# wsntxxn/TextToAudioGrounding

Hardware: AMD Instinct MI355X
Metric: clips/sec (10 s@32 kHz, 1-phrase) fwd+bwd (higher is better)
Workload: dtype f32

## Files before the change

### texttoaudiogrounding_amd/csrc/conv_wino.hip

```cpp
#include "conv_wino.h"

int tag_launch_gemm_batched(const float* A, int lda, long sA, const float* B, int ldb, long sB, float* C, int ldc, long sC, int M,
                            int N, int K, int batch, hipStream_t st, int transA);

namespace {

__device__ __forceinline__ f32x4 wino_prologue(f32x4 v, int mode, f32x4 s, f32x4 t) {
    if (mode == 1) {
        v.x = fmaxf(fmaf(v.x, s.x, t.x), 0.0f); v.y = fmaxf(fmaf(v.y, s.y, t.y), 0.0f);
        v.z = fmaxf(fmaf(v.z, s.z, t.z), 0.0f); v.w = fmaxf(fmaf(v.w, s.w, t.w), 0.0f);
    } else if (mode == 2) {
        v.x = fmaf(v.x > 0 ? v.x : 0.1f * v.x, s.x, t.x); v.y = fmaf(v.y > 0 ? v.y : 0.1f * v.y, s.y, t.y);
        v.z = fmaf(v.z > 0 ? v.z : 0.1f * v.z, s.z, t.z); v.w = fmaf(v.w > 0 ? v.w : 0.1f * v.w, s.w, t.w);
    } else if (mode == 3) {
        v.x = fmaf(v.x, s.x, t.x); v.y = fmaf(v.y, s.y, t.y); v.z = fmaf(v.z, s.z, t.z); v.w = fmaf(v.w, s.w, t.w);
    }
    return v;
}

__global__ __launch_bounds__(256) void wino_pack_kernel(const float* __restrict__ w, float* __restrict__ Uf,
                                                        float* __restrict__ Ud, int Cin, int Cout, int tiled_f, int tiled_d) {
    const long n = (long)Cin * Cout;
    for (long e = (long)blockIdx.x * 256 + threadIdx.x; e < n; e += (long)gridDim.x * 256) {
        const int co = (int)(e / Cin), ci = (int)(e % Cin);
// ... 318 lines not shown
        float q[3][4];
#pragma unroll
        for (int s = 0; s < 4; ++s) {
            const float hs = 0.5f * (u[1][s] + u[2][s]), hd = 0.5f * (u[1][s] - u[2][s]);
            q[0][s] = u[0][s] + hs;
            q[1][s] = hd;
            q[2][s] = hs + u[3][s];
        }
        float* o = dw + e * 9;
#pragma unroll
        for (int a = 0; a < 3; ++a) {
            const float hs = 0.5f * (q[a][1] + q[a][2]), hd = 0.5f * (q[a][1] - q[a][2]);
            o[3 * a + 0] = q[a][0] + hs;
            o[3 * a + 1] = hd;
            o[3 * a + 2] = hs + q[a][3];
        }
    }
}

struct WinoWgGeom { int th, tw; long T, Tpad; int S, kc; };
inline WinoWgGeom wino_wg_geom(int B, int H, int W, int Cin, int Cout) {
    WinoWgGeom g;
    g.th = (H + 1) / 2; g.tw = (W + 1) / 2;
    g.T = (long)B * g.th * g.tw;
    const long tiles = (long)((Cin + 127) / 128) * ((Cout + 127) / 128) * 16;
    long S = (1024 + tiles - 1) / tiles;
    if (S > g.T / 512) S = g.T / 512;
    if (S < 1) S = 1;
    long kc = (g.T + S - 1) / S;
    kc = (kc + 15) / 16 * 16;
    g.S = (int)((g.T + kc - 1) / kc);
    g.kc = (int)kc;
    g.Tpad = (long)g.S * kc;
    return g;
}

struct WinoGeom { int th, tw; long T; int G, P; };
inline WinoGeom wino_geom(int B, int H, int W, int Cout) {
    WinoGeom g;
    g.th = (H + 1) / 2; g.tw = (W + 1) / 2;
    g.T = (long)B * g.th * g.tw;
    g.G = 256 / (Cout / 4);
    const long per_wg = (long)g.G * WINO_ITERS;
    g.P = (int)((g.T + per_wg - 1) / per_wg) * g.G;
    return g;
}
inline bool wino_channels_ok(int C) { return C >= 32 && C <= 1024 && C % 4 == 0 && 256 % (C / 4) == 0; }

int wino_run(const float* x, const float* U, int pro, const float* s, const float* t, float* y, float* stats, const WinoEpi* epi,
             int B, int H, int W, int Cin, int Cout, float* ws, hipStream_t st, float* v_keep = nullptr) {
    if (wino_fused_ok(Cin, Cout)) {
        if (v_keep) {
            const WinoGeom gk = wino_geom(B, H, W, Cout);
            const int gk_in = (int)((gk.T * (Cin / 4) + 255) / 256);
            switch (pro) {
                case 0: hipLaunchKernelGGL(wino_input_kernel<0>, dim3(gk_in), dim3(256), 0, st, x, s, t, v_keep, B, H, W, Cin, gk.th, gk.tw, gk.T, gk.T); break;
                case 1: hipLaunchKernelGGL(wino_input_kernel<1>, dim3(gk_in), dim3(256), 0, st, x, s, t, v_keep, B, H, W, Cin, gk.th, gk.tw, gk.T, gk.T); break;
                case 2: hipLaunchKernelGGL(wino_input_kernel<2>, dim3(gk_in), dim3(256), 0, st, x, s, t, v_keep, B, H, W, Cin, gk.th, gk.tw, gk.T, gk.T); break;
                default: hipLaunchKernelGGL(wino_input_kernel<3>, dim3(gk_in), dim3(256), 0, st, x, s, t, v_keep, B, H, W, Cin, gk.th, gk.tw, gk.T, gk.T); break;
            }
        }
        return wino_fused_run(x, U, pro, s, t, y, stats, epi, B, H, W, Cin, Cout, st);
    }
    const WinoGeom g = wino_geom(B, H, W, Cout);
    float* V = v_keep ? v_keep : ws;
    float* Mb = v_keep ? ws : ws + (size_t)16 * g.T * Cin;
    const long items = g.T * (Cin / 4);
    const int gin = (int)((items + 255) / 256);
    switch (pro) {
        case 0: hipLaunchKernelGGL(wino_input_kernel<0>, dim3(gin), dim3(256), 0, st, x, s, t, V, B, H, W, Cin, g.th, g.tw, g.T, g.T); break;
        case 1: hipLaunchKernelGGL(wino_input_kernel<1>, dim3(gin), dim3(256), 0, st, x, s, t, V, B, H, W, Cin, g.th, g.tw, g.T, g.T); break;
        case 2: hipLaunchKernelGGL(wino_input_kernel<2>, dim3(gin), dim3(256), 0, st, x, s, t, V, B, H, W, Cin, g.th, g.tw, g.T, g.T); break;
        default: hipLaunchKernelGGL(wino_input_kernel<3>, dim3(gin), dim3(256), 0, st, x, s, t, V, B, H, W, Cin, g.th, g.tw, g.T, g.T); break;
    }
    tag_launch_gemm_batched(V, Cin, g.T * Cin, U, Cout, (long)Cin * Cout, Mb, Cout, g.T * Cout, (int)g.T, Cout, Cin, 16, st, 0);
    const int gout = g.P / g.G;
    const WinoEpi none{nullptr, nullptr, nullptr, nullptr, nullptr, 0, 0.0f, 0.0f, 0, 0, 0.0f, 0ull, 0};
    if (epi && epi->kind == 2)
        hipLaunchKernelGGL(wino_output_kernel<2>, dim3(gout), dim3(256), 0, st, Mb, y, stats, *epi, B, H, W, Cout, g.th, g.tw, g.T, g.P);
    else if (epi && epi->kind == 3)
        hipLaunchKernelGGL(wino_output_kernel<3>, dim3(gout), dim3(256), 0, st, Mb, y, stats, *epi, B, H, W, Cout, g.th, g.tw, g.T, g.P);
    else if (epi)
        hipLaunchKernelGGL(wino_output_kernel<1>, dim3(gout), dim3(256), 0, st, Mb, y, stats, *epi, B, H, W, Cout, g.th, g.tw, g.T, g.P);
    else
        hipLaunchKernelGGL(wino_output_kernel<0>, dim3(gout), dim3(256), 0, st, Mb, y, stats, none, B, H, W, Cout, g.th, g.tw, g.T, g.P);
    return 0;
}

}

extern "C" int tag_conv3x3_wino_ok(int B, int H, int W, int Cin, int Cout) {
    const bool fused = Cin % 64 == 0 && Cout % 64 == 0 && Cin >= 64 && Cout >= 64 && Cin <= 1024 && Cout <= 1024;
    if (!(B > 0 && H > 0 && W > 0 && (fused || (wino_channels_ok(Cin) && wino_channels_ok(Cout) && Cin % 32 == 0)))) return 0;
    const WinoGeom g = wino_geom(B, H, W, Cout);
    return g.T < (1L << 31) / 16 && (long)B * H * W < (1L << 31) && (long)B * H * W * (Cin > Cout ? Cin : Cout) < (1L << 29);
}

extern "C" int tag_pack_conv_weight_wino(const float* w, float* ufwd, float* udgrad, int Cin, int Cout, void* stream) {
    TAG_CHECK_ARG(w && (ufwd || udgrad) && Cin > 0 && Cout > 0);
    const long n = (long)Cin * Cout;
    hipLaunchKernelGGL(wino_pack_kernel, dim3(cdiv(n, 256) > 2048 ? 2048 : cdiv(n, 256)), dim3(256), 0, as_stream(stream), w, ufwd,
                       udgrad, Cin, Cout, wino_fused_ok(Cin, Cout) ? 1 : 0, wino_fused_ok(Cout, Cin) ? 1 : 0);
    TAG_LAUNCH_CHECK();
    return 0;
}

extern "C" size_t tag_conv3x3_wino_ws_bytes(int B, int H, int W, int Cin, int Cout) {
    if (wino_fused_ok(Cin > 0 ? Cin : 32, Cout)) return 64;
    const WinoGeom g = wino_geom(B, H, W, Cout);
    return (size_t)16 * g.T * ((size_t)Cin + Cout) * sizeof(float);
}

extern "C" int tag_conv3x3_wino_stats_rows(int B, int H, int W, int Cout) {
    if (wino_fused_ok(32, Cout)) return wino_fused_rows(B, H, W);
    if (!wino_channels_ok(Cout)) return 0;
    return wino_geom(B, H, W, Cout).P;
}

extern "C" int tag_conv3x3_wino_dgrad_poolsums(const float* dy, const float* u, float* dx, const float* yref, const float* bn_scale,
                                               const float* bn_shift, const float* bn_mean, const float* bn_invstd, float* bnpart,
                                               int B, int H, int W, int Cin, int Cout, int Hf, int Wf, int ph, int pw, int pool,
                                               float drop_p, uint64_t seed, void* ws, void* stream) {
    TAG_CHECK_ARG(dy && u && dx && yref && bn_scale && bn_shift && bn_mean && bn_invstd && bnpart && ws);
    TAG_CHECK_ARG(tag_conv3x3_wino_ok(B, H, W, Cin, Cout) && (long)B * Hf * Wf < (1L << 31));
    TAG_CHECK_ARG(pw == 2 && (ph == 1 || ph == 2) && H == Hf / ph && W == Wf / pw);
    TAG_CHECK_ARG((pool == 0 || pool == 2 || pool == 3) && drop_p >= 0.0f && drop_p < 1.0f);
    const float wavg = pool == 3 ? 0.0f : 1.0f / (float)(ph * pw), wmax = pool == 2 ? 0.0f : 1.0f;
    const WinoEpi epi{yref, bn_scale, bn_shift, bn_mean, bn_invstd, ph, wavg, wmax, Hf, Wf, drop_p, (unsigned long long)seed, 2};
    wino_run(dy, u, 0, nullptr, nullptr, dx, bnpart, &epi, B, H, W, Cin, Cout, static_cast<float*>(ws), as_stream(stream));
    TAG_LAUNCH_CHECK();
    return 0;
}

extern "C" size_t tag_conv3x3_wino_wgrad_ws_bytes(int B, int H, int W, int Cin, int Cout) {
    if (wino_fused_wgrad_ok(Cin, Cout)) return wino_fused_wgrad_ws_floats(B, H, W, Cin, Cout) * sizeof(float);
    const WinoWgGeom g = wino_wg_geom(B, H, W, Cin, Cout);
    return ((size_t)16 * g.Tpad * ((size_t)Cin + Cout) + (size_t)16 * g.S * Cin * Cout) * sizeof(float);
}

extern "C" int tag_conv3x3_wino_wgrad_can_reuse_v(int B, int H, int W, int Cin, int Cout) {
    if (wino_fused_wgrad_ok(Cin, Cout)) return 0;
    const WinoWgGeom g = wino_wg_geom(B, H, W, Cin, Cout);
    return g.Tpad == g.T;
}

extern "C" int tag_conv3x3_wino_wgrad(const float* x, int prologue, const float* in_scale, const float* in_shift, const float* dy,
                                      float* dw, int B, int H, int W, int Cin, int Cout, void* ws, const float* v_saved,
                                      void* stream) {
    TAG_CHECK_ARG((x || v_saved) && dy && dw && ws && tag_conv3x3_wino_ok(B, H, W, Cin, Cout));
    TAG_CHECK_ARG(v_saved == nullptr || tag_conv3x3_wino_wgrad_can_reuse_v(B, H, W, Cin, Cout));
    TAG_CHECK_ARG(prologue >= 0 && prologue <= 3 && (prologue == 0 || (in_scale && in_shift)));
    hipStream_t st = as_stream(stream);
    if (wino_fused_wgrad_ok(Cin, Cout) && x) {
        wino_fused_wgrad_run(x, prologue, in_scale, in_shift, dy, dw, B, H, W, Cin, Cout, static_cast<float*>(ws), st);
        TAG_LAUNCH_CHECK();
        return 0;
    }
    const WinoWgGeom g = wino_wg_geom(B, H, W, Cin, Cout);
    float* D = v_saved ? static_cast<float*>(ws) : static_cast<float*>(ws) + (size_t)16 * g.Tpad * Cin;
    const float* V = v_saved ? v_saved : static_cast<const float*>(ws);
    float* Vw = static_cast<float*>(ws);
    float* Pp = D + (size_t)16 * g.Tpad * Cout;
    const int gin = (int)((g.Tpad * (Cin / 4) + 255) / 256), gdy = (int)((g.Tpad * (Cout / 4) + 255) / 256);
    if (!v_saved) switch (prologue) {
        case 0: hipLaunchKernelGGL(wino_input_kernel<0>, dim3(gin), dim3(256), 0, st, x, in_scale, in_shift, Vw, B, H, W, Cin, g.th, g.tw, g.T, g.Tpad); break;
        case 1: hipLaunchKernelGGL(wino_input_kernel<1>, dim3(gin), dim3(256), 0, st, x, in_scale, in_shift, Vw, B, H, W, Cin, g.th, g.tw, g.T, g.Tpad); break;
        case 2: hipLaunchKernelGGL(wino_input_kernel<2>, dim3(gin), dim3(256), 0, st, x, in_scale, in_shift, Vw, B, H, W, Cin, g.th, g.tw, g.T, g.Tpad); break;
        default: hipLaunchKernelGGL(wino_input_kernel<3>, dim3(gin), dim3(256), 0, st, x, in_scale, in_shift, Vw, B, H, W, Cin, g.th, g.tw, g.T, g.Tpad); break;
    }
    hipLaunchKernelGGL(wino_dy_kernel, dim3(gdy), dim3(256), 0, st, dy, D, B, H, W, Cout, g.th, g.tw, g.T, g.Tpad);
    tag_launch_gemm_batched(D, Cout, (long)g.kc * Cout, V, Cin, (long)g.kc * Cin, Pp, Cin, (long)Cin * Cout, Cout, Cin, g.kc,
                            16 * g.S, st, 1);
    const long n = (long)Cin * Cout;
    hipLaunchKernelGGL(wino_wgrad_finish_kernel, dim3(cdiv(n, 256) > 4096 ? 4096 : cdiv(n, 256)), dim3(256), 0, st, Pp, g.S, Cin, Cout,
                       dw);
    TAG_LAUNCH_CHECK();
    return 0;
}

extern "C" int tag_conv3x3_wino_forward(const float* x, const float* u, int prologue, const float* in_scale,
                                        const float* in_shift, float* y, float* stats, int B, int H, int W, int Cin, int Cout,
                                        void* ws, float* v_keep, void* stream) {
    TAG_CHECK_ARG(x && u && y && ws && tag_conv3x3_wino_ok(B, H, W, Cin, Cout));
    TAG_CHECK_ARG(prologue >= 0 && prologue <= 3 && (prologue == 0 || (in_scale && in_shift)));
    wino_run(x, u, prologue, in_scale, in_shift, y, stats, nullptr, B, H, W, Cin, Cout, static_cast<float*>(ws), as_stream(stream),
             v_keep);
    TAG_LAUNCH_CHECK();
    return 0;
}

extern "C" int tag_conv3x3_wino_forward_bnrelu_pool_eval(const float* x, const float* u, int prologue, const float* in_scale,
                                                         const float* in_shift, float* out, const float* bn_scale,
                                                         const float* bn_shift, int B, int H, int W, int Cin, int Cout, int ph, int pw,
                                                         int pool, void* ws, void* stream) {
    TAG_CHECK_ARG(x && u && out && bn_scale && bn_shift && ws && tag_conv3x3_wino_ok(B, H, W, Cin, Cout));
    TAG_CHECK_ARG(prologue >= 0 && prologue <= 3 && (prologue == 0 || (in_scale && in_shift)));
    TAG_CHECK_ARG(pw == 2 && (ph == 1 || ph == 2) && H / ph > 0 && W >= 2 && (pool == 0 || pool == 2 || pool == 3));
    const float wavg = pool == 3 ? 0.0f : 1.0f / (float)(ph * pw), wmax = pool == 2 ? 0.0f : 1.0f;
    const WinoEpi epi{nullptr, bn_scale, bn_shift, nullptr, nullptr, ph, wavg, wmax, 0, 0, 0.0f, 0ull, 3};
    wino_run(x, u, prologue, in_scale, in_shift, out, nullptr, &epi, B, H, W, Cin, Cout, static_cast<float*>(ws), as_stream(stream));
    TAG_LAUNCH_CHECK();
    return 0;
}

extern "C" int tag_conv3x3_wino_dgrad_bnsums(const float* dy, const float* u, float* da, const float* yref, const float* bn_scale,
                                             const float* bn_shift, const float* bn_mean, const float* bn_invstd, float* bnpart,
                                             int B, int H, int W, int Cin, int Cout, void* ws, void* stream) {
    TAG_CHECK_ARG(dy && u && da && yref && bn_scale && bn_shift && bn_mean && bn_invstd && bnpart && ws);
    TAG_CHECK_ARG(tag_conv3x3_wino_ok(B, H, W, Cin, Cout));
    const WinoEpi epi{yref, bn_scale, bn_shift, bn_mean, bn_invstd, 0, 0.0f, 0.0f, 0, 0, 0.0f, 0ull, 1};
    wino_run(dy, u, 0, nullptr, nullptr, da, bnpart, &epi, B, H, W, Cin, Cout, static_cast<float*>(ws), as_stream(stream));
    TAG_LAUNCH_CHECK();
    return 0;
}
```

### texttoaudiogrounding_amd/csrc/conv_wino_fused.hip

```cpp
#include <type_traits>
#include "conv_wino.h"

#ifndef TAG_WG_ABL
#define TAG_WG_ABL 0
#endif
#ifndef TAG_WF_ABL
#define TAG_WF_ABL 0
#endif

namespace {

constexpr int FPL = 64 * 8 + 8;
constexpr int FBUF = 16 * FPL;
constexpr int FPARK_LD = 68;
constexpr int FPARK = 2 * 4 * 64 * FPARK_LD;
constexpr int FRED = 32 * 16 * 8 + 32;
constexpr int FLDS = FPARK + FRED;
constexpr int FSS = 4 * FBUF;
constexpr int FGM = 8;
static_assert(FSS + 2048 <= FLDS, "scale/shift staging must fit");

template <int PRO>
__device__ __forceinline__ f32x4 fused_prologue(f32x4 v, f32x4 s, f32x4 t) {
    if (PRO == 1) {
        v.x = fmaxf(fmaf(v.x, s.x, t.x), 0.0f); v.y = fmaxf(fmaf(v.y, s.y, t.y), 0.0f);
        v.z = fmaxf(fmaf(v.z, s.z, t.z), 0.0f); v.w = fmaxf(fmaf(v.w, s.w, t.w), 0.0f);
    } else if (PRO == 2) {
        v.x = fmaf(v.x > 0 ? v.x : 0.1f * v.x, s.x, t.x); v.y = fmaf(v.y > 0 ? v.y : 0.1f * v.y, s.y, t.y);
        v.z = fmaf(v.z > 0 ? v.z : 0.1f * v.z, s.z, t.z); v.w = fmaf(v.w > 0 ? v.w : 0.1f * v.w, s.w, t.w);
    } else if (PRO == 3) {
        v.x = fmaf(v.x, s.x, t.x); v.y = fmaf(v.y, s.y, t.y); v.z = fmaf(v.z, s.z, t.z); v.w = fmaf(v.w, s.w, t.w);
    }
    return v;
}

#define TAG_QUAD_FMAC(NAME, PERM)                                                                                             \
    __device__ __forceinline__ void NAME(const float (&t)[4], float f, f32x4& v) {                                           \
        float a = t[0], b = t[1], c = t[2], d = t[3];                                                                        \
        asm("s_nop 1\n\t"                                                                                                    \
            "v_fmac_f32_dpp %0, %0, %4 quad_perm:" PERM " row_mask:0xf bank_mask:0xf bound_ctrl:1\n\t"                       \
            "v_fmac_f32_dpp %1, %1, %4 quad_perm:" PERM " row_mask:0xf bank_mask:0xf bound_ctrl:1\n\t"                       \
            "v_fmac_f32_dpp %2, %2, %4 quad_perm:" PERM " row_mask:0xf bank_mask:0xf bound_ctrl:1\n\t"                       \
            "v_fmac_f32_dpp %3, %3, %4 quad_perm:" PERM " row_mask:0xf bank_mask:0xf bound_ctrl:1"                            \
            : "+v"(a), "+v"(b), "+v"(c), "+v"(d)                                                                             \
            : "v"(f));                                                                                                       \
        v = (f32x4){a, b, c, d};                                                                                             \
    }
TAG_QUAD_FMAC(quad_fmac_2211, "[2,2,1,1]")
TAG_QUAD_FMAC(quad_fmac_0033, "[0,0,3,3]")
#undef TAG_QUAD_FMAC

template <int HH>
__device__ __forceinline__ void fused_out_quad(const f32x16 (&acc)[8], int rq, f32x4 (&o)[4]) {
    f32x4 p0[4], p1[4];
#pragma unroll
    for (int s = 0; s < 4; ++s)
#pragma unroll
        for (int k = 0; k < 4; ++k) {
            const float m0 = acc[s][4 * rq + k], m1 = acc[4 + s][4 * rq + k];
            if (HH == 0) { p0[s][k] = m0 + m1; p1[s][k] = m1; }
            else { p0[s][k] = m0; p1[s][k] = -m0 - m1; }
        }
    o[0] = p0[0] + p0[1] + p0[2];
    o[1] = p0[1] - p0[2] + p0[3];
    o[2] = p1[0] + p1[1] + p1[2];
    o[3] = p1[1] - p1[2] + p1[3];
}

template <int PRO, int EPI>
__global__ __launch_bounds__(512) void wino_fused_kernel(const float* __restrict__ x, const float* __restrict__ U,
                                                         const float* __restrict__ in_scale, const float* __restrict__ in_shift,
                                                         float* __restrict__ y, float* __restrict__ stats, WinoEpi epi, int B, int H,
                                                         int W, int Cin, int Cout, int th, int tw, long T, int m_tiles, int n_tiles) {
    extern __shared__ __attribute__((aligned(16))) float smem[];
    const int tid = threadIdx.x, lane = tid & 63, wave = tid >> 6;
#ifdef TAG_WF_PROF
    const unsigned long long pt0 = __builtin_readcyclecounter();
#endif
    int mt, nt;
    {
        const int L = xcd_remap(blockIdx.x, m_tiles * n_tiles);
        const int gsz = FGM * n_tiles, g = L / gsz, rem = L - g * gsz;
        const int mcount = (m_tiles - g * FGM) < FGM ? (m_tiles - g * FGM) : FGM;
        nt = rem / mcount;
        mt = g * FGM + (rem - nt * mcount);
    }
    const long m0 = (long)mt * 64;
    const int n0 = nt * 64;
    const int nch = Cin >> 3;

    const int s = tid & 3, q = (tid >> 2) & 1, tl = tid >> 3;
    const float fb = s == 1 ? 1.0f : -1.0f;
    const __amdgpu_buffer_rsrc_t xrs = __builtin_amdgcn_make_buffer_rsrc(const_cast<float*>(x), 0, (int)((size_t)B * H * W * Cin * 4), 0x00020000);
    unsigned xo[4];
    float okb[4];
    bool okr[4];
    {
        const unsigned t = (unsigned)m0 + (unsigned)tl;
        const bool okt = t < (unsigned)T;
        const unsigned tt_ = okt ? t : 0u;
        const unsigned bi = tt_ / (unsigned)tw;
        const int j = (int)(tt_ - bi * (unsigned)tw);
        const int b = (int)(bi / (unsigned)th), i = (int)(bi - (unsigned)b * (unsigned)th);
        const int w = 2 * j - 1 + s;
        const bool okw = okt && (unsigned)w < (unsigned)W;
#pragma unroll
        for (int r = 0; r < 4; ++r) {
            const int h = 2 * i - 1 + r;
            okr[r] = okw && (unsigned)h < (unsigned)H;
            okb[r] = okr[r] ? INFINITY : 0.0f;
            xo[r] = okr[r] ? (unsigned)(((((size_t)b * H + h) * W + w) * Cin + 4 * q) * sizeof(float)) : 0x80000000u;
        }
    }
    const int vw0 = s * FPL + tl * 8 + ((q ^ ((tl >> 3) & 1)) << 2);

    const __amdgpu_buffer_rsrc_t urs = __builtin_amdgcn_make_buffer_rsrc(const_cast<float*>(U), 0, (int)((size_t)16 * Cin * Cout * 4), 0x00020000);
    const int un = (tid & 127) >> 1, uslot = tid & 1;
    const unsigned uo0 = (unsigned)((((tid >> 7) * 64 + un) * 8 + ((uslot ^ ((un >> 3) & 1)) << 2)) * sizeof(float));
    const int uw0 = (tid >> 7) * FPL + un * 8 + (uslot << 2);
    const unsigned ublk = (unsigned)__builtin_amdgcn_readfirstlane((int)((unsigned)nt * (unsigned)nch));

    const int hh = wave >> 2, wm = (wave >> 1) & 1, wn = wave & 1;
    const int kl = lane >> 5, ml = lane & 31;
    const int fsw = (kl ^ ((ml >> 3) & 1)) << 2;
    const int aoff = 2 * FBUF + 8 * hh * FPL + (wm * 32 + ml) * 8 + fsw;
    const int boff = 8 * hh * FPL + (wn * 32 + ml) * 8 + fsw;

    f32x16 acc[8];
    f32x4 xr[4], ur[4];
    auto load_x = [&](int c, int r) {
        xr[r] = __builtin_bit_cast(f32x4, __builtin_amdgcn_raw_buffer_load_b128(xrs, xo[r], c * 32, 0));
    };
    auto load_u = [&](int c, int i) {
        ur[i] = __builtin_bit_cast(f32x4, __builtin_amdgcn_raw_buffer_load_b128(urs, uo0 + i * (4 * 64 * 8 * 4), (ublk + c) * (16 * 64 * 8 * 4), 0));
    };
    f32x4 d[4], vv;
    float tt[4][4];
    f32x4 psc = {1.0f, 1.0f, 1.0f, 1.0f}, psh = {0.0f, 0.0f, 0.0f, 0.0f};
    auto ld_ss = [&](int c) {
        if (PRO != 0) {
            psc = *reinterpret_cast<const f32x4*>(smem + FSS + c * 8 + 4 * q);
            psh = *reinterpret_cast<const f32x4*>(smem + FSS + Cin + c * 8 + 4 * q);
        }
    };
    auto x_row = [&](int r) {
        if (TAG_WF_ABL & 4) return;
        if (PRO == 0) {
            d[r] = xr[r];
        } else if (PRO == 1) {
#pragma unroll
            for (int k = 0; k < 4; ++k) d[r][k] = __builtin_amdgcn_fmed3f(fmaf(xr[r][k], psc[k], psh[k]), 0.0f, okb[r]);
        } else {
// ... 492 lines not shown
        quad_fmac_2211(tt[r], fb, vv);
#endif
        *reinterpret_cast<f32x4*>(Vb + vw0 + 4 * r * FPL) = vv;
    };
    auto g_rows = [&]() {
#pragma unroll
        for (int k = 0; k < 4; ++k) {
            R[0][k] = gr[0][k];
            R[1][k] = gr[0][k] + gr[1][k];
            R[2][k] = gr[0][k] - gr[1][k];
            R[3][k] = gr[1][k];
        }
    };
    auto d_write = [&](float* Db, int r) {
#if TAG_WG_ABL & 2
        vv = gr[r & 1];
#else
        quad_fmac_0033(R[r], cb, vv);
#endif
        *reinterpret_cast<f32x4*>(Db + vw0 + 4 * r * FPL) = vv;
    };
    auto rotate_ok = [&]() {
        if (PRO != 0) {
#pragma unroll
            for (int r = 0; r < 4; ++r) okc[r] = okn[r];
        }
    };

    {
        f32x4 x0[4], g0[2];
        float ok0[4];
        col_offsets();
#pragma unroll
        for (int r = 0; r < 4; ++r) load_x(r);
        load_g(0); load_g(1);
        advance();
#pragma unroll
        for (int r = 0; r < 4; ++r) { x0[r] = xr[r]; ok0[r] = okn[r]; }
        g0[0] = gr[0]; g0[1] = gr[1];
        col_offsets();
#pragma unroll
        for (int r = 0; r < 4; ++r) load_x(r);
        load_g(0); load_g(1);
        advance();
        f32x4 x1[4], g1[2];
        float ok1[4];
#pragma unroll
        for (int r = 0; r < 4; ++r) { x1[r] = xr[r]; ok1[r] = okn[r]; xr[r] = x0[r]; okc[r] = ok0[r]; }
        g1[0] = gr[0]; g1[1] = gr[1]; gr[0] = g0[0]; gr[1] = g0[1];
#pragma unroll
        for (int r = 0; r < 4; ++r) x_row(r);
        x_col();
        g_rows();
#pragma unroll
        for (int r = 0; r < 4; ++r) { v_write(smem, r); d_write(smem + 2 * FBUF, r); }
#pragma unroll
        for (int r = 0; r < 4; ++r) { xr[r] = x1[r]; okn[r] = ok1[r]; }
        gr[0] = g1[0]; gr[1] = g1[1];
    }
    __syncthreads();

    int aJ[8], bJ[8];
#pragma unroll
    for (int j = 0; j < 8; ++j) {
        aJ[j] = aoff + j * FPL;
        bJ[j] = boff + j * FPL;
        asm volatile("" : "+v"(aJ[j]), "+v"(bJ[j]));
    }
#define WG_M4(J)                                                                                              \
    _Pragma("unroll") for (int e = 0; e < 4; ++e)                                                             \
        acc[J] = __builtin_amdgcn_mfma_f32_32x32x2f32(cur[aJ[J] + 128 * e], cur[bJ[J] + 128 * e], acc[J], 0, 0, 0)
#define WG_SB __builtin_amdgcn_sched_barrier(0)
    auto chunk = [&](auto stage) {
        constexpr int ST = decltype(stage)::value;
        const float* cur = smem + ST * FBUF;
        float* nxt = smem + (1 - ST) * FBUF;
        WG_SB;
        WG_M4(0); WG_SB; rotate_ok(); x_row(0); x_row(1); WG_SB;
        WG_M4(1); WG_SB; x_row(2); x_row(3); x_col(); WG_SB;
        WG_M4(2); WG_SB; v_write(nxt, 0); v_write(nxt, 1); col_offsets(); load_x(0); load_x(1); WG_SB;
        WG_M4(3); WG_SB; v_write(nxt, 2); v_write(nxt, 3); load_x(2); load_x(3); WG_SB;
        WG_M4(4); WG_SB; g_rows(); d_write(nxt + 2 * FBUF, 0); d_write(nxt + 2 * FBUF, 1); WG_SB;
        WG_M4(5); WG_SB; d_write(nxt + 2 * FBUF, 2); d_write(nxt + 2 * FBUF, 3); load_g(0); load_g(1); advance(); WG_SB;
        WG_M4(6); WG_SB;
        WG_M4(7); WG_SB;
        __syncthreads();
    };
    {
        int c = 0;
        for (; c + 1 < cps; c += 2) {
            chunk(std::integral_constant<int, 0>{});
            chunk(std::integral_constant<int, 1>{});
        }
        if (c < cps) chunk(std::integral_constant<int, 0>{});
    }
#undef WG_M4
#undef WG_SB

    float* pb = part + ((size_t)(sl * 2 + hh) * Cout + cob * 64 + wn * 32 + ml) * Cin * 9 + (size_t)(cib * 64 + wm * 32 + 4 * kl) * 9;
#pragma unroll
    for (int rq = 0; rq < 4; ++rq) {
        float o[4][9];
#pragma unroll
        for (int k = 0; k < 4; ++k) {
            float P[3][4];
#pragma unroll
            for (int sx = 0; sx < 4; ++sx) {
                const float m0 = acc[sx][4 * rq + k], m1 = acc[4 + sx][4 * rq + k];
                if (hh == 0) { P[0][sx] = m0 + 0.5f * m1; P[1][sx] = 0.5f * m1; P[2][sx] = 0.5f * m1; }
                else { P[0][sx] = 0.5f * m0; P[1][sx] = -0.5f * m0; P[2][sx] = 0.5f * m0 - m1; }
            }
#pragma unroll
            for (int a = 0; a < 3; ++a) {
                const float hs = 0.5f * (P[a][1] + P[a][2]), hd = 0.5f * (P[a][1] - P[a][2]);
                o[k][3 * a + 0] = P[a][0] + hs;
                o[k][3 * a + 1] = hd;
                o[k][3 * a + 2] = hs + P[a][3];
            }
        }
        float* q = pb + (size_t)(8 * rq) * 9;
        const float* of = &o[0][0];
#pragma unroll
        for (int v4 = 0; v4 < 9; ++v4) *reinterpret_cast<f32x4*>(q + 4 * v4) = (f32x4){of[4 * v4], of[4 * v4 + 1], of[4 * v4 + 2], of[4 * v4 + 3]};
    }
}

template <int Q>
__global__ __launch_bounds__(256) void wino_fused_wgrad_finish_kernel(const float* __restrict__ part, int nshare, long n4, float* __restrict__ dw) {
    constexpr int E = 256 / Q;
    __shared__ f32x4 run[Q > 1 ? 256 : 1];
    const int el = threadIdx.x % E, q = threadIdx.x / E;
    const int per = (nshare + Q - 1) / Q;
    const int p0 = q * per, p1 = (p0 + per < nshare) ? p0 + per : nshare;
    for (long e0 = (long)blockIdx.x * E; e0 < n4; e0 += (long)gridDim.x * E) {
        const long e = e0 + el;
        f32x4 a = {0.0f, 0.0f, 0.0f, 0.0f};
        if (e < n4)
            for (int p = p0; p < p1; ++p) a += *reinterpret_cast<const f32x4*>(part + ((size_t)p * n4 + e) * 4);
        if (Q == 1) {
            if (e < n4) *reinterpret_cast<f32x4*>(dw + e * 4) = a;
        } else {
            run[threadIdx.x] = a;
            __syncthreads();
            if (q == 0 && e < n4) {
#pragma unroll
                for (int k = 1; k < Q; ++k) a += run[k * E + el];
                *reinterpret_cast<f32x4*>(dw + e * 4) = a;
            }
            __syncthreads();
        }
    }
}

}

bool wino_fused_ok(int Cin, int Cout) { return Cin >= 8 && Cin % 8 == 0 && Cin <= 1024 && Cout >= 64 && Cout % 64 == 0; }

int wino_fused_rows(int B, int H, int W) {
    const long T = (long)B * ((H + 1) / 2) * ((W + 1) / 2);
    return (int)((T + 63) / 64);
}

int wino_fused_run(const float* x, const float* U, int pro, const float* s, const float* t, float* y, float* stats, const WinoEpi* epi,
                   int B, int H, int W, int Cin, int Cout, hipStream_t st) {
    const WinoEpi none{nullptr, nullptr, nullptr, nullptr, nullptr, 0, 0.0f, 0.0f, 0, 0, 0.0f, 0ull, 0};
    const int kind = epi ? epi->kind : 0;
    const WinoEpi& e = epi ? *epi : none;
#define FUSED_CASE(P_, E_) launch_fused<P_, E_>(x, U, s, t, y, stats, e, B, H, W, Cin, Cout, st); return 0
    if (kind == 0) {
        switch (pro) { case 0: FUSED_CASE(0, 0); case 1: FUSED_CASE(1, 0); case 2: FUSED_CASE(2, 0); default: FUSED_CASE(3, 0); }
    }
    if (kind == 3) {
        switch (pro) { case 0: FUSED_CASE(0, 3); case 1: FUSED_CASE(1, 3); case 2: FUSED_CASE(2, 3); default: FUSED_CASE(3, 3); }
    }
    if (pro != 0) return -1;
    if (kind == 1) { FUSED_CASE(0, 1); }
    FUSED_CASE(0, 2);
#undef FUSED_CASE
}

bool wino_fused_wgrad_ok(int Cin, int Cout) { return Cin >= 64 && Cin % 64 == 0 && Cout >= 64 && Cout % 64 == 0; }

size_t wino_fused_wgrad_ws_floats(int B, int H, int W, int Cin, int Cout) {
    const WgGeom g = wg_geom(B, H, W, Cin, Cout);
    return (size_t)2 * g.S * Cin * Cout * 9;
}

int wino_fused_wgrad_run(const float* x, int pro, const float* s, const float* t, const float* dy, float* dw, int B, int H, int W,
                         int Cin, int Cout, float* ws, hipStream_t st) {
    const WgGeom g = wg_geom(B, H, W, Cin, Cout);
    const int grid = g.nci * g.nco * g.S;
    const size_t lds = (size_t)4 * FBUF * sizeof(float);
#define WG_CASE(P_)                                                                                                          \
    {                                                                                                                        \
        static bool attr_set = false;                                                                                        \
        if (!attr_set) {                                                                                                     \
            (void)hipFuncSetAttribute(reinterpret_cast<const void*>(&wino_fused_wgrad_kernel<P_>),                           \
                                      hipFuncAttributeMaxDynamicSharedMemorySize, (int)lds);                                 \
            attr_set = true;                                                                                                 \
        }                                                                                                                    \
        hipLaunchKernelGGL((wino_fused_wgrad_kernel<P_>), dim3(grid), dim3(512), lds, st, x, s, t, dy, ws, B, H, W, Cin, Cout, g.th,  \
                           g.tw, g.nci, g.nco, g.S, g.cps);                                                                  \
    }
    switch (pro) {
        case 0: WG_CASE(0) break;
        case 1: WG_CASE(1) break;
        case 2: WG_CASE(2) break;
        default: WG_CASE(3) break;
    }
#undef WG_CASE
    const long n4 = (long)Cin * Cout * 9 / 4;
    const auto blocks = [&](int e) { const long b = cdiv(n4, (long)e); return dim3((unsigned)(b > 4096 ? 4096 : b)); };
    if (n4 >= 131072 || g.S < 8) hipLaunchKernelGGL(wino_fused_wgrad_finish_kernel<1>, blocks(256), dim3(256), 0, st, ws, 2 * g.S, n4, dw);
    else if (n4 >= 32768 || g.S < 32) hipLaunchKernelGGL(wino_fused_wgrad_finish_kernel<4>, blocks(64), dim3(256), 0, st, ws, 2 * g.S, n4, dw);
    else hipLaunchKernelGGL(wino_fused_wgrad_finish_kernel<16>, blocks(16), dim3(256), 0, st, ws, 2 * g.S, n4, dw);
    return 0;
}
```

Baseline: 1987.

## Add row-split Winograd weight-gradient kernel for 128-aligned channel counts

After: 2045, median of 6. +2.9%, better.

```diff
diff --git a/texttoaudiogrounding_amd/csrc/conv_wino.hip b/texttoaudiogrounding_amd/csrc/conv_wino.hip
--- a/texttoaudiogrounding_amd/csrc/conv_wino.hip
+++ b/texttoaudiogrounding_amd/csrc/conv_wino.hip
@@ -494,7 +494,10 @@
     TAG_CHECK_ARG(prologue >= 0 && prologue <= 3 && (prologue == 0 || (in_scale && in_shift)));
     hipStream_t st = as_stream(stream);
     if (wino_fused_wgrad_ok(Cin, Cout) && x) {
-        wino_fused_wgrad_run(x, prologue, in_scale, in_shift, dy, dw, B, H, W, Cin, Cout, static_cast<float*>(ws), st);
+        if (wino_fused_wgrad_run(x, prologue, in_scale, in_shift, dy, dw, B, H, W, Cin, Cout, static_cast<float*>(ws), st) != 0) {
+            tag_set_error("%s:%d: the weight-gradient kernel's LDS limit could not be set on this device", __FILE__, __LINE__);
+            return TAG_EINVAL;
+        }
         TAG_LAUNCH_CHECK();
         return 0;
     }
diff --git a/texttoaudiogrounding_amd/csrc/conv_wino_fused.hip b/texttoaudiogrounding_amd/csrc/conv_wino_fused.hip
--- a/texttoaudiogrounding_amd/csrc/conv_wino_fused.hip
+++ b/texttoaudiogrounding_amd/csrc/conv_wino_fused.hip
@@ -1,3 +1,4 @@
+#include <atomic>
 #include <type_traits>
 #include "conv_wino.h"
 
@@ -796,6 +797,307 @@
     }
 }
 
+constexpr int RPL = 8 * 128 + 8;
+constexpr int RBUF = 4 * RPL;
+
+inline bool wg_rows_ok(int Cin, int Cout) { return Cin % 128 == 0 && Cout % 128 == 0; }
+
+template <int PRO, int R0>
+__device__ __forceinline__ void wgrad_rows_body(float* smem, const float* __restrict__ x, const float* __restrict__ in_scale,
+                                                const float* __restrict__ in_shift, const float* __restrict__ dy,
+                                                float* __restrict__ part, int B, int H, int W, int Cin, int Cout, int th, int tw,
+                                                int sl, int cib, int cob, int cps) {
+    constexpr int RA = R0 == 0 ? 0 : (R0 == 2 ? 2 : 1);
+    constexpr int RB = R0 == 0 ? 2 : (R0 == 1 ? 2 : (R0 == 2 ? 1 : 3));
+    constexpr int NG = (R0 == 1 || R0 == 2) ? 2 : 1;
+    constexpr int GA = R0 == 3 ? 1 : 0;
+    const int tid = threadIdx.x, lane = tid & 63;
+    const int wave = __builtin_amdgcn_readfirstlane(tid >> 6);
+    const int s = lane & 3, quad = lane >> 2;
+    const float fb = s == 1 ? 1.0f : -1.0f;
+    const float cb = s == 1 ? 1.0f : (s == 2 ? -1.0f : 0.0f);
+    const int xbytes = (int)(((size_t)B * H * W + 1) * Cin * 4), dbytes = (int)((size_t)B * H * W * Cout * 4);
+    const unsigned xvo = (unsigned)((s * Cin + cib * 128 + 4 * quad) * 4);
+    const unsigned dvo = (unsigned)(((s & 1) * Cout + cob * 128 + 4 * quad) * 4);
+    const int vw0 = s * RPL + wave * 128 + 4 * quad;
+    int tb, ti, tj;
+    {
+        const unsigned t = (unsigned)sl * (unsigned)cps * 8u + (unsigned)wave;
+        const unsigned bi = t / (unsigned)tw;
+        tj = (int)(t - bi * (unsigned)tw);
+        tb = (int)(bi / (unsigned)th);
+        ti = (int)(bi - (unsigned)tb * (unsigned)th);
+        tb = __builtin_amdgcn_readfirstlane(tb); ti = __builtin_amdgcn_readfirstlane(ti); tj = __builtin_amdgcn_readfirstlane(tj);
+    }
+    auto advance = [&]() {
+        tj += 8;
+        while (tj >= tw) { tj -= tw; ++ti; }
+        while (ti >= th) { ti -= th; ++tb; }
+    };
+    f32x4 psc[2], psh[2];
+#pragma unroll
+    for (int i = 0; i < 2; ++i) {
+        psc[i] = (f32x4){1.0f, 1.0f, 1.0f, 1.0f}; psh[i] = (f32x4){0.0f, 0.0f, 0.0f, 0.0f};
+        if (PRO != 0) {
+            psc[i] = *reinterpret_cast<const f32x4*>(in_scale + cib * 128 + 64 * i + 4 * quad);
+            psh[i] = *reinterpret_cast<const f32x4*>(in_shift + cib * 128 + 64 * i + 4 * quad);
+        }
+    }
+
+    const int sp = wave & 3, cih = wave >> 2;
+    const int kl = lane >> 5, ml = lane & 31;
+    int ab = sp * RPL + kl * 128 + cih * 64 + ml;
+    int bb = 2 * RBUF + sp * RPL + kl * 128 + ml;
+    asm volatile("" : "+v"(ab), "+v"(bb));
+
+    f32x16 acc[8];
+#pragma unroll
+    for (int i = 0; i < 8; ++i)
+#pragma unroll
+        for (int r = 0; r < 16; ++r) acc[i][r] = 0.0f;
+
+    f32x4 xr[2][2], gr[2][NG];
+    float okn[2] = {0.0f, 0.0f}, okc[2];
+    unsigned xcol = 0x80000000u, gcol = 0x80000000u;
+    float xclamp = 0.0f;
+    auto col_offsets = [&]() {
+        const bool cx = (unsigned)(2 * tj - 1 + s) < (unsigned)W;
+        xcol = cx ? xvo : 0x80000000u;
+        gcol = (2 * tj + (s & 1)) < W ? dvo : 0x80000000u;
+        if (PRO != 0) xclamp = cx ? INFINITY : 0.0f;
+    };
+    auto load_x = [&](int j) {
+        const int h = 2 * ti - 1 + (j == 0 ? RA : RB);
+        const bool rv = tb < B && (unsigned)h < (unsigned)H;
+        const int so = (int)(((unsigned)(tb * H + h) * (unsigned)W + 2u * (unsigned)tj) * (unsigned)(Cin * 4));
+        const __amdgpu_buffer_rsrc_t rs = __builtin_amdgcn_make_buffer_rsrc(const_cast<float*>(x) - Cin, 0, rv ? xbytes : 0, 0x00020000);
+        xr[0][j] = __builtin_bit_cast(f32x4, __builtin_amdgcn_raw_buffer_load_b128(rs, xcol, so, 0));
+        xr[1][j] = __builtin_bit_cast(f32x4, __builtin_amdgcn_raw_buffer_load_b128(rs, xcol + 256u, so, 0));
+        if (PRO != 0) okn[j] = rv ? xclamp : 0.0f;
+    };
+    auto load_g = [&](int j) {
+        const int h = 2 * ti + GA + j;
+        const bool rv = tb < B && h < H;
+        const int so = (int)(((unsigned)(tb * H + h) * (unsigned)W + 2u * (unsigned)tj) * (unsigned)(Cout * 4));
+        const __amdgpu_buffer_rsrc_t rs = __builtin_amdgcn_make_buffer_rsrc(const_cast<float*>(dy), 0, rv ? dbytes : 0, 0x00020000);
+        gr[0][j] = __builtin_bit_cast(f32x4, __builtin_amdgcn_raw_buffer_load_b128(rs, gcol, so, 0));
+        gr[1][j] = __builtin_bit_cast(f32x4, __builtin_amdgcn_raw_buffer_load_b128(rs, gcol + 256u, so, 0));
+    };
+    f32x4 d[2][2], vv;
+    float tt[2][4], R[2][4];
+    auto x_row = [&](int i, int j) {
+        if (PRO == 0) {
+            d[i][j] = xr[i][j];
+        } else if (PRO == 1) {
+#pragma unroll
+            for (int k = 0; k < 4; ++k) d[i][j][k] = __builtin_amdgcn_fmed3f(fmaf(xr[i][j][k], psc[i][k], psh[i][k]), 0.0f, okc[j]);
+        } else {
+            const f32x4 v = fused_prologue<PRO>(xr[i][j], psc[i], psh[i]);
+            d[i][j] = okc[j] > 0.0f ? v : (f32x4){0.0f, 0.0f, 0.0f, 0.0f};
+        }
+    };
+    auto x_col = [&](int i) {
+#pragma unroll
+        for (int k = 0; k < 4; ++k) tt[i][k] = R0 == 1 ? d[i][0][k] + d[i][1][k] : d[i][0][k] - d[i][1][k];
+    };
+    auto v_write = [&](float* Vb, int i) {
+        quad_fmac_2211(tt[i], fb, vv);
+        *reinterpret_cast<f32x4*>(Vb + vw0 + 64 * i) = vv;
+    };
+    auto g_rows = [&](int i) {
+#pragma unroll
+        for (int k = 0; k < 4; ++k) {
+            if (NG == 1) R[i][k] = gr[i][0][k];
+            else R[i][k] = R0 == 1 ? gr[i][0][k] + gr[i][NG - 1][k] : gr[i][0][k] - gr[i][NG - 1][k];
+        }
+    };
+    auto d_write = [&](float* Db, int i) {
+        quad_fmac_0033(R[i], cb, vv);
+        *reinterpret_cast<f32x4*>(Db + vw0 + 64 * i) = vv;
+    };
+    auto rotate_ok = [&]() {
+        if (PRO != 0) { okc[0] = okn[0]; okc[1] = okn[1]; }
+    };
+    auto load_chunk = [&]() {
+        col_offsets();
+        load_x(0); load_x(1);
+#pragma unroll
+        for (int j = 0; j < NG; ++j) load_g(j);
+        advance();
+    };
+
+    {
+        f32x4 x0[2][2], g0[2][NG], x1[2][2], g1[2][NG];
+        float ok0[2], ok1[2];
+        load_chunk();
+#pragma unroll
+        for (int i = 0; i < 2; ++i) {
+#pragma unroll
+            for (int j = 0; j < 2; ++j) x0[i][j] = xr[i][j];
+#pragma unroll
+            for (int j = 0; j < NG; ++j) g0[i][j] = gr[i][j];
+        }
+        ok0[0] = okn[0]; ok0[1] = okn[1];
+        load_chunk();
+#pragma unroll
+        for (int i = 0; i < 2; ++i) {
+#pragma unroll
+            for (int j = 0; j < 2; ++j) { x1[i][j] = xr[i][j]; xr[i][j] = x0[i][j]; }
+#pragma unroll
+            for (int j = 0; j < NG; ++j) { g1[i][j] = gr[i][j]; gr[i][j] = g0[i][j]; }
+        }
+#pragma unroll
+        for (int j = 0; j < 2; ++j) { ok1[j] = okn[j]; okc[j] = ok0[j]; }
+#pragma unroll
+        for (int i = 0; i < 2; ++i) {
+            x_row(i, 0); x_row(i, 1); x_col(i); g_rows(i);
+            v_write(smem, i); d_write(smem + 2 * RBUF, i);
+        }
+#pragma unroll
+        for (int i = 0; i < 2; ++i) {
+#pragma unroll
+            for (int j = 0; j < 2; ++j) xr[i][j] = x1[i][j];
+#pragma unroll
+            for (int j = 0; j < NG; ++j) gr[i][j] = g1[i][j];
+        }
+        okn[0] = ok1[0]; okn[1] = ok1[1];
+    }
+    __syncthreads();
+
+    float fA[2][2], fB[2][4];
+#define WR_FRAG(E)                                                                                            \
+    do {                                                                                                      \
+        fA[(E) & 1][0] = cur[ab + 256 * (E)]; fA[(E) & 1][1] = cur[ab + 32 + 256 * (E)];                      \
+        _Pragma("unroll") for (int b = 0; b < 4; ++b) fB[(E) & 1][b] = cur[bb + 32 * b + 256 * (E)];          \
+    } while (0)
+#define WR_M4(E, A_)                                                                                          \
+    _Pragma("unroll") for (int b = 0; b < 4; ++b)                                                             \
+        acc[4 * (A_) + b] = __builtin_amdgcn_mfma_f32_32x32x2f32(fA[(E) & 1][A_], fB[(E) & 1][b], acc[4 * (A_) + b], 0, 0, 0)
+#define WR_SB __builtin_amdgcn_sched_barrier(0)
+    auto chunk = [&](auto stage) {
+        constexpr int ST = decltype(stage)::value;
+        const float* cur = smem + ST * RBUF;
+        float* nxt = smem + (1 - ST) * RBUF;
+        WR_SB;
+        WR_FRAG(0); WR_SB;
+        WR_M4(0, 0); WR_SB; rotate_ok(); x_row(0, 0); x_row(0, 1); x_row(1, 0); x_row(1, 1); x_col(0); x_col(1); WR_SB;
+        WR_FRAG(1); WR_M4(0, 1); WR_SB; v_write(nxt, 0); v_write(nxt, 1); WR_SB;
+        WR_M4(1, 0); WR_SB; col_offsets(); load_x(0); load_x(1); WR_SB;
+        WR_FRAG(2); WR_M4(1, 1); WR_SB; g_rows(0); g_rows(1); d_write(nxt + 2 * RBUF, 0); WR_SB;
+        WR_M4(2, 0); WR_SB; d_write(nxt + 2 * RBUF, 1);
+        _Pragma("unroll") for (int j = 0; j < NG; ++j) load_g(j);
+        advance(); WR_SB;
+        WR_FRAG(3); WR_M4(2, 1); WR_SB;
+        WR_M4(3, 0); WR_SB;
+        WR_M4(3, 1); WR_SB;
+        __syncthreads();
+    };
+    {
+        int c = 0;
+        for (; c + 1 < cps; c += 2) {
+            chunk(std::integral_constant<int, 0>{});
+            chunk(std::integral_constant<int, 1>{});
+        }
+        if (c < cps) chunk(std::integral_constant<int, 0>{});
+    }
+#undef WR_FRAG
+#undef WR_M4
+#undef WR_SB
+
+    float* pb = part + (((size_t)sl * 16 + 4 * R0 + sp) * Cout + cob * 128 + ml) * Cin + cib * 128 + cih * 64 + 4 * kl;
+#pragma unroll
+    for (int a = 0; a < 2; ++a)
+#pragma unroll
+        for (int b = 0; b < 4; ++b)
+#pragma unroll
+            for (int rq = 0; rq < 4; ++rq)
+                *reinterpret_cast<f32x4*>(pb + (size_t)(32 * b) * Cin + 32 * a + 8 * rq) =
+                    (f32x4){acc[4 * a + b][4 * rq], acc[4 * a + b][4 * rq + 1], acc[4 * a + b][4 * rq + 2], acc[4 * a + b][4 * rq + 3]};
+}
+
+template <int PRO>
+__global__ __launch_bounds__(512) void wino_fused_wgrad_rows_kernel(const float* __restrict__ x, const float* __restrict__ in_scale,
+                                                                    const float* __restrict__ in_shift, const float* __restrict__ dy,
+                                                                    float* __restrict__ part, int B, int H, int W, int Cin, int Cout,
+                                                                    int th, int tw, int nci, int nco, int S, int cps) {
+    extern __shared__ __attribute__((aligned(16))) float smem[];
+    const int per = nci * nco * 4;
+    const int L = xcd_remap(blockIdx.x, per * S);
+    const int sl = L / per;
+    const int rem = L - sl * per;
+    const int r0 = rem & 3, blk = rem >> 2;
+    const int cib = blk / nco, cob = blk - cib * nco;
+#define WR_CASE(R_) wgrad_rows_body<PRO, R_>(smem, x, in_scale, in_shift, dy, part, B, H, W, Cin, Cout, th, tw, sl, cib, cob, cps)
+    switch (r0) {
+        case 0: WR_CASE(0); break;
+        case 1: WR_CASE(1); break;
+        case 2: WR_CASE(2); break;
+        default: WR_CASE(3); break;
+    }
+#undef WR_CASE
+}
+
+template <int Q>
+__global__ __launch_bounds__(256) void wino_fused_wgrad_rows_finish_kernel(const float* __restrict__ part, int nshare, long n,
+                                                                           float* __restrict__ dw) {
+    constexpr int E = 256 / Q;
+    __shared__ float run[Q > 1 ? 256 * 9 : 1];
+    const int el = threadIdx.x % E, q = threadIdx.x / E;
+    const int per = (nshare + Q - 1) / Q;
+    const int p0 = q * per, p1 = (p0 + per < nshare) ? p0 + per : nshare;
+    for (long e0 = (long)blockIdx.x * E; e0 < n; e0 += (long)gridDim.x * E) {
+        const long e = e0 + el;
+        float a[9];
+#pragma unroll
+        for (int j = 0; j < 9; ++j) a[j] = 0.0f;
+        if (e < n)
+            for (int p = p0; p < p1; ++p) {
+                const int hh = p & 1;
+                const float* m = part + (size_t)((p >> 1) * 16 + 8 * hh) * n + e;
+                float P[3][4];
+#pragma unroll
+                for (int sx = 0; sx < 4; ++sx) {
+                    const float m0 = m[(size_t)sx * n], m1 = m[(size_t)(4 + sx) * n];
+                    if (hh == 0) { P[0][sx] = m0 + 0.5f * m1; P[1][sx] = 0.5f * m1; P[2][sx] = 0.5f * m1; }
+                    else { P[0][sx] = 0.5f * m0; P[1][sx] = -0.5f * m0; P[2][sx] = 0.5f * m0 - m1; }
+                }
+#pragma unroll
+                for (int t = 0; t < 3; ++t) {
+                    const float hs = 0.5f * (P[t][1] + P[t][2]), hd = 0.5f * (P[t][1] - P[t][2]);
+                    a[3 * t + 0] += P[t][0] + hs;
+                    a[3 * t + 1] += hd;
+                    a[3 * t + 2] += hs + P[t][3];
+                }
+            }
+        if (Q > 1) {
+#pragma unroll
+            for (int j = 0; j < 9; ++j) run[j * 256 + threadIdx.x] = a[j];
+            __syncthreads();
+            if (q == 0) {
+#pragma unroll
+                for (int k = 1; k < Q; ++k)
+#pragma unroll
+                    for (int j = 0; j < 9; ++j) a[j] += run[j * 256 + k * E + el];
+            }
+            __syncthreads();
+        }
+        if (q == 0 && e < n) {
+#pragma unroll
+            for (int j = 0; j < 9; ++j) dw[e * 9 + j] = a[j];
+        }
+    }
+}
+
+inline int wg_set_lds(const void* fn, size_t bytes, std::atomic<unsigned long long>& done) {
+    int dev = 0;
+    if (hipGetDevice(&dev) != hipSuccess || dev < 0 || dev >= 64) return -1;
+    if (!(done.load(std::memory_order_acquire) >> dev & 1ull)) {
+        if (hipFuncSetAttribute(fn, hipFuncAttributeMaxDynamicSharedMemorySize, (int)bytes) != hipSuccess) return -1;
+        done.fetch_or(1ull << dev, std::memory_order_release);
+    }
+    return 0;
+}
+
 }
 
 bool wino_fused_ok(int Cin, int Cout) { return Cin >= 8 && Cin % 8 == 0 && Cin <= 1024 && Cout >= 64 && Cout % 64 == 0; }
@@ -834,17 +1136,20 @@
                          int Cin, int Cout, float* ws, hipStream_t st) {
     const WgGeom g = wg_geom(B, H, W, Cin, Cout);
     const int grid = g.nci * g.nco * g.S;
-    const size_t lds = (size_t)4 * FBUF * sizeof(float);
+    const bool rows = wg_rows_ok(Cin, Cout);
+    const size_t lds = (size_t)4 * (rows ? RBUF : FBUF) * sizeof(float);
 #define WG_CASE(P_)                                                                                                          \
     {                                                                                                                        \
-        static bool attr_set = false;                                                                                        \
-        if (!attr_set) {                                                                                                     \
-            (void)hipFuncSetAttribute(reinterpret_cast<const void*>(&wino_fused_wgrad_kernel<P_>),                           \
-                                      hipFuncAttributeMaxDynamicSharedMemorySize, (int)lds);                                 \
-            attr_set = true;                                                                                                 \
+        static std::atomic<unsigned long long> set_full{0}, set_rows{0};                                                     \
+        if (rows) {                                                                                                          \
+            if (wg_set_lds(reinterpret_cast<const void*>(&wino_fused_wgrad_rows_kernel<P_>), lds, set_rows) != 0) return -1; \
+            hipLaunchKernelGGL((wino_fused_wgrad_rows_kernel<P_>), dim3(grid), dim3(512), lds, st, x, s, t, dy, ws, B, H, W, Cin,   \
+                               Cout, g.th, g.tw, g.nci / 2, g.nco / 2, g.S, g.cps);                                          \
+        } else {                                                                                                             \
+            if (wg_set_lds(reinterpret_cast<const void*>(&wino_fused_wgrad_kernel<P_>), lds, set_full) != 0) return -1;      \
+            hipLaunchKernelGGL((wino_fused_wgrad_kernel<P_>), dim3(grid), dim3(512), lds, st, x, s, t, dy, ws, B, H, W, Cin, Cout,  \
+                               g.th, g.tw, g.nci, g.nco, g.S, g.cps);                                                        \
         }                                                                                                                    \
-        hipLaunchKernelGGL((wino_fused_wgrad_kernel<P_>), dim3(grid), dim3(512), lds, st, x, s, t, dy, ws, B, H, W, Cin, Cout, g.th,  \
-                           g.tw, g.nci, g.nco, g.S, g.cps);                                                                  \
     }
     switch (pro) {
         case 0: WG_CASE(0) break;
@@ -854,9 +1159,14 @@
     }
 #undef WG_CASE
     const long n4 = (long)Cin * Cout * 9 / 4;
-    const auto blocks = [&](int e) { const long b = cdiv(n4, (long)e); return dim3((unsigned)(b > 4096 ? 4096 : b)); };
-    if (n4 >= 131072 || g.S < 8) hipLaunchKernelGGL(wino_fused_wgrad_finish_kernel<1>, blocks(256), dim3(256), 0, st, ws, 2 * g.S, n4, dw);
-    else if (n4 >= 32768 || g.S < 32) hipLaunchKernelGGL(wino_fused_wgrad_finish_kernel<4>, blocks(64), dim3(256), 0, st, ws, 2 * g.S, n4, dw);
-    else hipLaunchKernelGGL(wino_fused_wgrad_finish_kernel<16>, blocks(16), dim3(256), 0, st, ws, 2 * g.S, n4, dw);
+    const int Q = (n4 >= 131072 || g.S < 8) ? 1 : ((n4 >= 32768 || g.S < 32) ? 4 : 16);
+    const auto blocks = [&](long n, int e) { const long b = cdiv(n, (long)e); return dim3((unsigned)(b > 4096 ? 4096 : b)); };
+    if (rows) {
+        const long n = (long)Cin * Cout;
+        if (Q == 1) hipLaunchKernelGGL(wino_fused_wgrad_rows_finish_kernel<1>, blocks(n, 256), dim3(256), 0, st, ws, 2 * g.S, n, dw);
+        else hipLaunchKernelGGL(wino_fused_wgrad_rows_finish_kernel<4>, blocks(n, 64), dim3(256), 0, st, ws, 2 * g.S, n, dw);
+    } else if (Q == 1) hipLaunchKernelGGL(wino_fused_wgrad_finish_kernel<1>, blocks(n4, 256), dim3(256), 0, st, ws, 2 * g.S, n4, dw);
+    else if (Q == 4) hipLaunchKernelGGL(wino_fused_wgrad_finish_kernel<4>, blocks(n4, 64), dim3(256), 0, st, ws, 2 * g.S, n4, dw);
+    else hipLaunchKernelGGL(wino_fused_wgrad_finish_kernel<16>, blocks(n4, 16), dim3(256), 0, st, ws, 2 * g.S, n4, dw);
     return 0;
 }
```
